# bitmagier/q-learning

Hardware: AMD Instinct MI355X
Metric: env-steps/sec + grad-updates/sec, Breakout 84×84×4, 1/2/4/8 MI355X (higher is better)
Workload: dtype fp32; 1 GPU; C3: 8192 Breakout envs per GPU, replay 1000000 per GPU in HBM (prefilled), Nature-DQN (3 conv + 2 dense) in fp32, B=1024, update every 128 env-steps per GPU (replay ratio 8 samples/env-step), epsilon-greedy acting; envs_per_gpu=8192, batch=1024, replay_capacity=1000000, update_after_actions=128, parallelism=single, rccl_world=1, global_batch_per_update=1024, env_dtype=fp32 physics, u8 frames, qnet_dtype=fp32 (exact-fp32 MFMA v_mfma_f32_16x16x4_f32)

## Files before the change

q-learning_amd/csrc/qnet32.hip:

```cpp
#include <hip/hip_ext.h>
#include <hip/hip_runtime.h>

#include <algorithm>
#include <cmath>
#include <cstdlib>
#include <map>
#include <tuple>
#include <vector>

#include "objects.h"
#include "profiler.h"
#include "qnet.h"
#include "qnet32_kernels.h"
#include "update32_dev.h"

namespace qlx {

using namespace q32;

struct F32Net {
  bool bg_rows = true;
  int c1_skip = 1;
  bool update_scheduled = false;
  bool dense_partials = false;
// ... 591 lines not shown
    if (e && atoi(e) > 0) {
      n = atoi(e);
    } else {
      int dev = 0;
      QLX_HIP(hipGetDevice(&dev));
      QLX_HIP(hipDeviceGetAttribute(&n, hipDeviceAttributeMultiprocessorCount, dev));
    }
  }
  return n;
}

static Grid grid(int M, int BM, int N, int BN, int nz) { return Grid{(M + BM - 1) / BM, (N + BN - 1) / BN, nz}; }

static int c1_skip(const qlx_model* m) { return m->fp32->c1_skip; }

static int balanced_whole_tiles(int M) {
  const int ncu = num_cus(), t = M / 64, whole = t - t % ncu;
  if (whole < ncu || M - whole * 64 > 32 * ncu) return 0;
  return whole;
}

template <class P, class S>
static void launch_list(qlx_model* m, const P& p, const S& side, const char* scope, double work, hipStream_t s) {
  hipEvent_t ea = nullptr, eb = nullptr;
  if (m->prof) m->prof->ext(scope, work, &ea, &eb);
  const size_t lds = std::max(gemm_lds_bytes<P>(), S::LDS);
  hipExtLaunchKernelGGL((k_gemm32_side<P, S>), dim3(side.blocks() + p.g.blocks()), dim3(threads_of<P>()), lds, s, ea, eb, 0u, p, side);
  QLX_HIP(hipGetLastError());
  debug_sync(s, scope);
}

static bool bg_rows(const qlx_model* m) { return m->fp32->bg_rows; }

static bool c1_sparse_dz(const qlx_model* m) { return bg_rows(m) && c1_skip(m); }
template <class PW, class PR, class PF>
static void conv_fwd(qlx_model* m, int M, const float* in, const float* wt, const float* bias, float* out, const char* scope,
                     double work, hipStream_t s, const PF& plain) {
  const int whole = balanced_whole_tiles(M);
  if (!whole) {
    launch(m, plain, scope, work, s);
    return;
  }
  const PW pw{Grid{whole, 1, 1}, in, wt, bias, out, M};
  const PR pr{{Grid{(M - whole * 64 + 15) / 16, 1, 1}, in, wt, bias, out, M}, whole * 4};
  launch_pair(m, pw, pr, NoSide{}, scope, work, s);
}

void f32_forward(qlx_model* m, const uint8_t* const* table, int B, hipStream_t s) {
  F32Net& w = *m->fp32;
  QLX_CHECK(m->ws_batch >= B, QLX_E_STATE, "f32 forward: workspace too small");
  m->last_batch = B;
  const float* p = m->d_params;
  for (int c0 = 0; c0 < B; c0 += w.fchunk) {
    const int n = std::min(w.fchunk, B - c0);
    const bool big = n > 2048;
    const bool lists = bg_rows(m);
    unsigned long long* cnt = w.frcnt + 2 * kListSlots * kCntStride * w.fparity;
    const bool one = c1_one(n);
    const int G = c1_grid(n);
    const int per_slot = ((G + kListSlots - 1) / kListSlots) * ((n + G - 1) / G);
    const int cap2 = per_slot * 81, cap3 = per_slot * 49;
    QLX_CHECK((size_t)kListSlots * cap2 <= w.frl_cap * 81, QLX_E_STATE, "row lists too small");
    const C1Lists L{lists ? w.frl2 : nullptr, w.frl3, cap2, cap3, cnt, w.frcnt + 2 * kListSlots * kCntStride * (w.fparity ^ 1),
                    w.fbgc, w.fsteps, w.fneed, w.fneed_ld, w.frows2, w.fbg2, w.frows3, w.fbg3};
    if (lists) w.fparity ^= 1;
    {
      const char* sc = big ? "f32_conv1_fwd_big" : "f32_conv1_fwd";
      hipEvent_t ea = nullptr, eb = nullptr;
      if (m->prof) m->prof->ext(sc, 2.0 * n * 400 * 32 * 256, &ea, &eb);
      auto kern = one ? k_conv1_fwd32<0, true> : k_conv1_fwd32<1>;
      QLX_CHECK((n + G - 1) / G <= (one ? 1 : kC1MaxIt), QLX_E_STATE, "conv1 forward: too many samples per block");
      const size_t frames = (one ? 1 : 2) * kC1Frames;
      const size_t lds = frames + 3 * kC1RmDw * 4 + (size_t)((n + G - 1) / G) * 6 * 8 + 8;
      set_lds_limit((const void*)kern, frames + 3 * kC1RmDw * 4 + (size_t)(one ? 1 : kC1MaxIt) * 6 * 8 + 8);
      hipExtLaunchKernelGGL(kern, dim3(G), dim3(256), lds, s, ea, eb, 0u, table + (size_t)c0 * 4, n,
                            p + var_offset(0), p + var_offset(1), w.fa1, c1_skip(m), L);
      QLX_HIP(hipGetLastError());
      debug_sync(s, sc);
    }
    if (lists) {
      const int nw = std::min(256, std::max(16, n / 16));
      float* c2 = w.fbgc + 32;
      float* c3 = w.fbgc + 96;
      const BgRows2 s23{{nw, w.frl2, cnt, cap2, c2, w.fa2}, {nw, w.frl3, cnt + kCntStride, cap3, c3, w.fa3}};
      auto lgrid = [&](int cap, int BM, int BN) { return Grid{1 + kListSlots * ((cap + BM - 1) / BM), 64 / BN, 1}; };
      auto run = [&](auto t2, auto t3, const char* sc2, const char* sc3) {
        using P2 = decltype(t2);
        using P3 = decltype(t3);
        const ConstRows cr{{w.fbgc, p + var_offset(2), p + var_offset(3), c2}, {c2, p + var_offset(4), p + var_offset(5), c3}};
        P2 p2{lgrid(cap2, P2::BM, P2::BN), w.fa1, p + var_offset(2), p + var_offset(3), w.fa2, w.frl2, cap2, cnt, w.fbgc};
        p2.pre_batched = big;
        launch_list(m, p2, cr, sc2, 2.0 * n * 81 * 64 * 512, s);
        launch_list(m, P3{lgrid(cap3, P3::BM, P3::BN), w.fa2, p + var_offset(4), p + var_offset(5), w.fa3, w.frl3, cap3, cnt + kCntStride, c2},
                    s23, sc3, 2.0 * n * 49 * 64 * 576, s);
      };
      if (big) {
        run(PConv2FwdL<64, 64, 2, 2>{}, PConv3FwdL<64, 64, 2, 2>{}, "f32_conv2_fwd_big", "f32_conv3_fwd_big");
        launch(m, PFc1FwdB{grid(n, PFc1FwdB::BM, 512, PFc1FwdB::BN, 1), w.fa3, p + var_offset(6), p + var_offset(7), w.fa4 + (size_t)c0 * 512, n}, "f32_fc1_fwd_big",
               2.0 * n * 3136 * 512, s);
      } else {
        run(PConv2FwdL<64, 64, 2, 2>{}, PConv3FwdL<32, 64, 2, 2>{}, "f32_conv2_fwd", "f32_conv3_fwd");
        launch(m, PFc1FwdS{grid(n, PFc1FwdS::BM, 512, PFc1FwdS::BN, 1), w.fa3, p + var_offset(6), p + var_offset(7), w.fa4 + (size_t)c0 * 512, n}, "f32_fc1_fwd",
               2.0 * n * 3136 * 512, s);
      }
    } else if (big) {
      launch(m, PConv2Fwd{grid(n * 81, 64, 64, 64, 1), w.fa1, p + var_offset(2), p + var_offset(3), w.fa2, n * 81}, "f32_conv2_fwd_big",
             2.0 * n * 81 * 64 * 512, s);
      launch(m, PConv3Fwd{grid(n * 49, 64, 64, 64, 1), w.fa2, p + var_offset(4), p + var_offset(5), w.fa3, n * 49}, "f32_conv3_fwd_big",
             2.0 * n * 49 * 64 * 576, s);
      launch(m, PFc1FwdB{grid(n, PFc1FwdB::BM, 512, PFc1FwdB::BN, 1), w.fa3, p + var_offset(6), p + var_offset(7), w.fa4 + (size_t)c0 * 512, n}, "f32_fc1_fwd_big",
             2.0 * n * 3136 * 512, s);
    } else {
      conv_fwd<PConv2Fwd, PConv2FwdR>(m, n * 81, w.fa1, p + var_offset(2), p + var_offset(3), w.fa2, "f32_conv2_fwd", 2.0 * n * 81 * 64 * 512, s,
                                      PConv2FwdS{grid(n * 81, 64, 64, 32, 1), w.fa1, p + var_offset(2), p + var_offset(3), w.fa2, n * 81});
      conv_fwd<PConv3Fwd, PConv3FwdR>(m, n * 49, w.fa2, p + var_offset(4), p + var_offset(5), w.fa3, "f32_conv3_fwd", 2.0 * n * 49 * 64 * 576, s,
                                      PConv3FwdS{grid(n * 49, 64, 64, 32, 1), w.fa2, p + var_offset(4), p + var_offset(5), w.fa3, n * 49});
      launch(m, PFc1FwdS{grid(n, PFc1FwdS::BM, 512, PFc1FwdS::BN, 1), w.fa3, p + var_offset(6), p + var_offset(7), w.fa4 + (size_t)c0 * 512, n}, "f32_fc1_fwd",
             2.0 * n * 3136 * 512, s);
    }
  }
}

void f32_head(int mode, const Fc2Args& a, int B, hipStream_t s) {
  constexpr int kHs3 = 4;
  const dim3 g((B + 15) / 16), blk(256);
  switch (mode) {
    case 0: hipLaunchKernelGGL(k_head32<0>, g, blk, 0, s, a); break;
    case 1: hipLaunchKernelGGL(k_head32<1>, g, blk, 0, s, a); break;
    case 2: hipLaunchKernelGGL(k_head32<2>, g, blk, 0, s, a); break;
    default: hipLaunchKernelGGL((k_head32<3, kHs3>), dim3((B + kHs3 - 1) / kHs3), blk, 0, s, a); break;
  }
  QLX_HIP(hipGetLastError());
  debug_sync(s, "k_head32");
}

Fc2Args f32_fc2_args(qlx_model* m, int B) {
  Fc2Args a = fc2_common(m, B);
  a.a4f = m->fp32->fa4;
  return a;
}

template <class Side>
static void f32_fc1_bwd(qlx_model* m, int B, const Side& S, hipStream_t s) {
  F32Net& w = *m->fp32;
  float* G = m->d_grads;
  const float* p = m->d_params;
  PFc1WgradS Pw{grid(3136, PFc1WgradS::BM, 512, PFc1WgradS::BN, 1), w.fa3, w.fdz4, G + var_offset(6), G + var_offset(7), B};
  PFc1DgradS Pd{grid(B, PFc1DgradS::BM, 3136, PFc1DgradS::BN, 1), w.fdz4, p + var_offset(6), w.fa3, w.fdz3, B};
  if (bg_rows(m)) {
    Pd.pbg = w.fpbg3;
    Pd.bg = w.fbg3;
    Pd.bg_ld = w.fneed_ld;
  }
  launch_pair(m, Pw, Pd, S, "f32_fc1_bwd", 2.0 * 2.0 * B * 512 * 3136, s);
}

void f32_backward_dense(qlx_model* m, int B, const uint8_t* actions, const float* y, float* loss_dev, hipStream_t s,
                        const float* weights, float* td_abs) {
  F32Net& w = *m->fp32;
  QLX_CHECK(B <= w.fchunk && B == m->last_batch, QLX_E_STATE, "f32 backward: batch must follow its forward");
  w.dense_partials = false;
  f32_grad_workspace(m, B);
  float* G = m->d_grads;
  float *gs = m->w.gs, *hs = m->w.hs;
  {
    ProfScope ps(m->prof, "f32_head", s);
    Fc2Args a = f32_fc2_args(m, B);
    a.actions = actions;
    a.y = y;
    a.gsample = gs;
    a.hsample = hs;
    a.weights = weights;
    a.td_abs = td_abs;
    a.dz4_out = w.fdz4;
    f32_head(3, a, B, s);
  }
  f32_fc1_bwd(m, B, SideFc2{w.fa4, actions, gs, hs, B, G + var_offset(8), G + var_offset(9), loss_dev}, s);
}

const float* f32_a4(qlx_model* m) { return m->fp32->fa4; }

float* f32_dz4_begin(qlx_model* m, int B) {
  F32Net& w = *m->fp32;
  QLX_CHECK(B <= w.fchunk && B == m->last_batch, QLX_E_STATE, "f32 backward: batch must follow its forward");
// ... 251 lines not shown
```

q-learning_amd/csrc/qnet32_kernels.h:

```cpp
#pragma once
#include <hip/hip_runtime.h>

#include <cstdint>
#include <type_traits>

#include "qlx_internal.h"

namespace qlx {
namespace q32 {

typedef float f32x4 __attribute__((ext_vector_type(4)));

constexpr int BK = 32;
constexpr int kListSlots = 8;
constexpr int kCntStride = 16;

__host__ __device__ constexpr int kmaj_pad(int rows, int r) { return rows + ((r - rows % 64) % 64 + 64) % 64; }
__host__ __device__ constexpr int kmaj_pitch(int rows) {
  return kmaj_pad(rows, 48) < kmaj_pad(rows, 16) ? kmaj_pad(rows, 48) : kmaj_pad(rows, 16);
}
static_assert(kmaj_pitch(32) == 48 && kmaj_pitch(64) == 80 && kmaj_pitch(128) == 144, "KMAJ pitches");

template <int ROWS, bool KMAJ>
struct Opnd {
// ... 462 lines not shown
      }
    }
  }
}

template <class P>
__device__ __forceinline__ void body(const P& p, int lb, float* lds) { gemm_body(p, lb, lds); }

template <class P>
__global__ __launch_bounds__(threads_of<P>()) void k_gemm32(const P p) {
  extern __shared__ float lds[];
  body(p, block_order<P>(blockIdx.x, gridDim.x), lds);
}

constexpr int kPairMinW = 4;
template <class P, class = void>
struct MinWOf : std::integral_constant<int, 1> {};
template <class P>
struct MinWOf<P, std::void_t<decltype(P::MINW)>> : std::integral_constant<int, P::MINW> {};
template <class P, class = void>
struct HasMinW : std::false_type {};
template <class P>
struct HasMinW<P, std::void_t<decltype(P::MINW)>> : std::true_type {};
template <class P1, class P2>
constexpr int pair_minw() {
  return (HasMinW<P1>::value || HasMinW<P2>::value)
             ? (MinWOf<P1>::value > MinWOf<P2>::value ? MinWOf<P1>::value : MinWOf<P2>::value)
             : kPairMinW;
}
template <class P1, class P2, class S, class T>
__global__ __launch_bounds__(256, (pair_minw<P1, P2>())) void k_gemm32_pair(const P1 p1, const P2 p2, const S side, const T tail) {
  static_assert(KSplitOf<P1>::value == 1 && KSplitOf<P2>::value == 1, "pair launches: 256 threads");
  extern __shared__ float lds[];
  const int b = blockIdx.x, ns = side.blocks();
  if (b < ns) { side.run(b, lds); return; }
  const int h = b - ns;
  const int g1 = p1.g.blocks(), g2 = p2.g.blocks();
  if (h < g1) body(p1, block_order<P1>(h, g1), lds);
  else if (h < g1 + g2) body(p2, block_order<P2>(h - g1, g2), lds);
  else tail.run(h - g1 - g2, lds);
}

template <class P, class S>
__global__ __launch_bounds__(threads_of<P>()) void k_gemm32_side(const P p, const S side) {
  extern __shared__ float lds[];
  const int b = blockIdx.x, ns = side.blocks();
  if (b < ns) { side.run(b, lds); return; }
  body(p, block_order<P>(b - ns, (int)gridDim.x - ns), lds);
}

template <int P = 81>
struct SideBgSum {
  static constexpr size_t LDS = 4 * 64 * sizeof(float);
  static constexpr int Q = (P + 3) / 4;
  const float* pbg;
  float* S;
  int nz;
  __host__ __device__ int blocks() const { return nz; }
  __device__ void run(int z, float* lds) const {
    const int oc = threadIdx.x & 63, q = threadIdx.x >> 6, p0 = Q * q, n = q < 3 ? Q : P - 3 * Q;
    float v[Q];
#pragma unroll
    for (int i = 0; i < Q; ++i) v[i] = i < n ? pbg[((size_t)z * P + p0 + i) * 64 + oc] : 0.0f;
    float t = 0.0f;
#pragma unroll
    for (int i = 0; i < Q; ++i)
      if (i < n) t = __fadd_rn(t, v[i]);
    lds[q * 64 + oc] = t;
    __syncthreads();
    if (q == 0) S[(size_t)z * 64 + oc] = __fadd_rn(__fadd_rn(__fadd_rn(lds[oc], lds[64 + oc]), lds[128 + oc]), lds[192 + oc]);
  }
};

struct NoSide {
  static constexpr size_t LDS = 0;
  __host__ __device__ int blocks() const { return 0; }
  __device__ void run(int, float*) const {}
};


#define QLX_CONV_FWD_CHAINS 1
constexpr int kConvFwdChains = QLX_CONV_FWD_CHAINS;
static_assert(kConvFwdChains == 1, "conv forward policies: one chain per output");
template <int W, int C, int KS, int OC, int BM, int BN, int T, bool SEL = false>
struct ConvFwdStreams {
  using SA = AffineStream<BM, false, T>;
  using SB = AffineStream<BN, true, T>;
  SA a;
  SB b;
  uint32_t cxo[SA::N], msk[SA::N];
  struct Regs {
    typename SA::Regs a;
    typename SB::Regs b;
  };
  __device__ void load(int s, Regs& x) const {
    const int tap = (s * BK) / C, c0 = (s * BK) % C, kh = tap / KS, kw = tap - kh * KS;
    const uint32_t so = (uint32_t)((kh * W + kw) * C + c0) * 4u;
    if constexpr (SEL) {
#pragma unroll
      for (int i = 0; i < SA::N; ++i)
        if (SA::O::F4 % T == 0 || a.tid + i * T < SA::O::F4) {
          const bool cst = (msk[i] >> tap) & 1u;
          x.a[i] = buf_ld4(a.rs, cst ? cxo[i] + (uint32_t)c0 * 4u : a.vo[i] + so, 0u);
        }
    } else {
      a.load(so, 0, x.a);
    }
    b.load((uint32_t)s * BK * OC * 4u, 0, x.b);
  }
  __device__ void store(float* as, float* bs, const Regs& x) const {
    a.store(as, x.a);
    b.store(bs, x.b);
  }
  __device__ void init_b(const float* w, int col0, int tid) {
    b.init(w, (uint32_t)KS * KS * C * OC * 4u, tid, [col0](int r, int k) { return (uint32_t)(k * OC + col0 + r) * 4u; });
  }
};

template <int H, int W, int C, int KS, int S, int OH, int OW, int OC, int BM_ = 64, int BN_ = 64, int WM_ = 2, int WN_ = 2>
struct PConvFwd {
  static constexpr int BM = BM_, BN = BN_, WM = WM_, WN = WN_;
  static constexpr int MINW = 3;
  static constexpr bool LOAD_FENCE = !(H == 20 && BN_ == 64);
  static constexpr bool A_KMAJ = false, B_KMAJ = true, BIAS = false;
  Grid g;
  const float* in;
  const float* w;
  const float* bias;
  float* out;
  int M;
  __host__ __device__ void decode(int lb, int& tm, int& tn, int& z) const { g.decode(lb, tm, tn, z); }
  __host__ __device__ int nslabs(int) const { return KS * KS * C / BK; }
  using Streams = ConvFwdStreams<W, C, KS, OC, BM_, BN_, WM_ * WN_ * 64>;
  __device__ Streams streams(int, int row0, int col0, int tid) const {
    Streams st;
    const int m = M;
    st.a.init(in, (uint32_t)(M / (OH * OW)) * (uint32_t)(H * W * C * 4), tid, [row0, m](int r, int k) {
      const int row = row0 + r, b = row / (OH * OW), p = row - b * (OH * OW), oh = p / OW, ow = p - oh * OW;
      return row < m ? (uint32_t)(((b * H + oh * S) * W + ow * S) * C + k) * 4u : kOob;
    });
    st.init_b(w, col0, tid);
    return st;
  }
  __device__ void epi(int, int row, int col, f32x4 v) const {
#pragma unroll
    for (int r = 0; r < 4; ++r)
      if (row + r < M) out[(size_t)(row + r) * OC + col] = relu(v[r] + bias[col]);
  }
  __device__ f32x4 epi_pre(int, int, int col) const {
    const float b = bias[col];
    return f32x4{b, b, b, b};
  }
  __device__ void epi_post(int, int row, int col, f32x4 v, f32x4 b) const {
#pragma unroll
    for (int r = 0; r < 4; ++r)
      if (row + r < M) out[(size_t)(row + r) * OC + col] = relu(v[r] + b[r]);
  }
};
using PConv2Fwd = PConvFwd<20, 20, 32, 4, 2, 9, 9, 64>;
using PConv3Fwd = PConvFwd<9, 9, 64, 3, 1, 7, 7, 64>;
using PConv2FwdS = PConvFwd<20, 20, 32, 4, 2, 9, 9, 64, 64, 32, 2, 2>;
using PConv3FwdS = PConvFwd<9, 9, 64, 3, 1, 7, 7, 64, 64, 32, 2, 2>;
template <class Base>
struct RowShift : Base {
  int tm0;
  __host__ __device__ void decode(int lb, int& tm, int& tn, int& z) const {
    Base::decode(lb, tm, tn, z);
    tm += tm0;
  }
};
using PConv2FwdR = RowShift<PConvFwd<20, 20, 32, 4, 2, 9, 9, 64, 16, 64, 1, 4>>;
using PConv3FwdR = RowShift<PConvFwd<9, 9, 64, 3, 1, 7, 7, 64, 16, 64, 1, 4>>;

template <int H, int W, int C, int KS, int S, int OH, int OW, int OC, int BM_ = 64, int BN_ = 64, int WM_ = 2, int WN_ = 2,
          bool SEL = false>
struct PConvFwdL {
  static constexpr int BM = BM_, BN = BN_, WM = WM_, WN = WN_;
  static constexpr bool A_KMAJ = false, B_KMAJ = true, BIAS = false, RAW_ORDER = true;
  static constexpr bool LOAD_FENCE = true;
  static constexpr int R = OH * OW;
  using OA = Opnd<BM, false>;
  static constexpr int T = WM * WN * 64, NA = (OA::F4 + T - 1) / T;
  Grid g;
  const float* in;
  const float* w;
  const float* bias;
  float* out;
  const int* list;
  int cap;
  const unsigned long long* cnt;
  const float* cx;
  bool pre_batched = true;
  struct Pre { float b; int o[4]; };

  __host__ __device__ void decode(int lb, int& tm, int& tn, int& z) const { g.decode(lb, tm, tn, z); }
  __host__ __device__ int nslabs(int) const { return KS * KS * C / BK; }
  __device__ int count(int x) const { return (int)(cnt[x * 2 * kCntStride] >> 32); }
  template <int N>
  __device__ void entries(const int (&row)[N], int (&out)[N]) const {
    const int tm = q32_uniform(row[0] / BM);
    const int x = (tm - 1) % kListSlots, base = ((tm - 1) / kListSlots) * BM;
    const int n = count(x);
    int v[N];
#pragma unroll
    for (int i = 0; i < N; ++i) v[i] = list[x * cap + min(base + row[i] % BM, cap - 1)];
#pragma unroll
    for (int i = 0; i < N; ++i) out[i] = base + row[i] % BM < n ? v[i] : -1;
  }
  __device__ bool active(int, int row0) const {
    const int tm = row0 / BM;
    return tm != 0 && ((tm - 1) / kListSlots) * BM < count((tm - 1) % kListSlots);
  }
  __device__ Pre epi_pre(int, int row, int col) const {
    Pre q;
    q.b = bias[col];
    if (!pre_batched) {
#pragma unroll
    for (int r = 0; r < 4; ++r) {
      const int tm = (row + r) / BM;
      const int x = (tm - 1) % kListSlots, lr = ((tm - 1) / kListSlots) * BM + (row + r) % BM;
      q.o[r] = lr < count(x) ? list[x * cap + lr] : -1;
    }
    } else {
    const int rows[4] = {row, row + 1, row + 2, row + 3};
    entries(rows, q.o);
    }
    return q;
  }
  __device__ void epi_post(int, int, int col, f32x4 v, const Pre& q) const {
#pragma unroll
    for (int r = 0; r < 4; ++r)
      if (q.o[r] >= 0) out[(size_t)(q.o[r] & 0xFFFFF) * OC + col] = relu(v[r] + q.b);
  }
  using Streams = ConvFwdStreams<W, C, KS, OC, BM_, BN_, T, SEL>;
  __device__ Streams streams(int, int row0, int col0, int tid) const {
    Streams st;
    st.a.tid = tid;
    const char* lo = (const char*)in;
    const char* base = SEL && (const char*)cx < lo ? (const char*)cx : lo;
    const uint32_t in_off = (uint32_t)(lo - base), cx_off = SEL ? (uint32_t)((const char*)cx - base) : 0u;
    st.a.rs = buf_rsrc(base, kNoEnd);
    int rows[NA], raws[NA];
#pragma unroll
    for (int i = 0; i < NA; ++i) {
      int r = 0, k = 0;
      OA::coord(tid + i * T, r, k);
      rows[i] = row0 + r;
    }
    entries(rows, raws);
#pragma unroll
    for (int i = 0; i < NA; ++i) {
      int r = 0, k = 0;
      OA::coord(tid + i * T, r, k);
      const int raw = raws[i], e = raw >= 0 ? raw & 0xFFFFF : -1;
      const int bb = e / R, pp = e - bb * R, oh = pp / OW, ow = pp - oh * OW;
      st.a.vo[i] = e >= 0 ? in_off + (uint32_t)(((bb * H + oh * S) * W + ow * S) * C + k) * 4u : kOob;
      st.cxo[i] = cx_off + (uint32_t)k * 4u;
      st.msk[i] = SEL && raw >= 0 ? (uint32_t)raw >> 20 : 0u;
    }
    st.init_b(w, col0, tid);
    return st;
  }
};
template <int BM, int BN, int WM, int WN>
using PConv2FwdL = PConvFwdL<20, 20, 32, 4, 2, 9, 9, 64, BM, BN, WM, WN, false>;
template <int BM, int BN, int WM, int WN>
using PConv3FwdL = PConvFwdL<9, 9, 64, 3, 1, 7, 7, 64, BM, BN, WM, WN, true>;

template <int C, int KS, int OC>
struct PConstRow {
  static constexpr int BM = 16, BN = OC, WM = 1, WN = 4, T = 256;
  static constexpr bool A_KMAJ = false, B_KMAJ = true, BIAS = false;
  static constexpr Grid g{1, 1, 1};
  const float* cx;
  const float* w;
  const float* bias;
  float* cbuf;
  __host__ __device__ void decode(int, int& tm, int& tn, int& z) const { tm = tn = z = 0; }
  __host__ __device__ int nslabs(int) const { return KS * KS * C / BK; }
  __device__ float epi_pre(int, int, int col) const { return bias[col]; }
  __device__ void epi_post(int, int row, int col, f32x4 v, float b) const {
    if (row == 0) cbuf[col] = relu(v[0] + b);
  }
  struct Streams {
    AffineStream<BM, false, T> a;
    AffineStream<BN, true, T> b;
    struct Regs {
      typename AffineStream<BM, false, T>::Regs a;
      typename AffineStream<BN, true, T>::Regs b;
    };
    __device__ void load(int s, Regs& x) const {
      a.load((uint32_t)((s * BK) % C) * 4u, 0, x.a);
      b.load((uint32_t)s * BK * OC * 4u, 0, x.b);
    }
    __device__ void store(float* as, float* bs, const Regs& x) const {
      a.store(as, x.a);
      b.store(bs, x.b);
    }
  };
  __device__ Streams streams(int, int, int, int tid) const {
    Streams st;
    st.a.init(cx, (uint32_t)C * 4u, tid, [](int r, int k) { return r == 0 ? (uint32_t)k * 4u : kOob; });
    st.b.init(w, (uint32_t)KS * KS * C * OC * 4u, tid, [](int r, int k) { return (uint32_t)(k * OC + r) * 4u; });
    return st;
  }
};

struct ConstRows {
  using PA = PConstRow<32, 4, 64>;
  using PB = PConstRow<64, 3, 64>;
  static constexpr size_t LDS = gemm_lds_bytes<PA>();
  PA pa;
  PB pb;
  __host__ __device__ int blocks() const { return 1; }
  __device__ void run(int, float* lds) const {
    gemm_body(pa, 0, lds);
    __syncthreads();
    __threadfence();
    gemm_body(pb, 0, lds);
  }
};

struct BgRows {
  static constexpr size_t LDS = 64 * sizeof(float);
  static constexpr int U = 8;
  int nblk;
  const int* list;
  const unsigned long long* cnt;
  int cap;
  const float* c_in;
  float* out;
  __host__ __device__ int blocks() const { return nblk; }
  __device__ void run(int blk, float* lds) const {
    const int tid = threadIdx.x, q = tid & 15, RB = (int)blockDim.x >> 4;
    const f32x4 v = ld4(c_in + 4 * q);
    for (int x = 0; x < kListSlots; ++x) {
      const int nbg = (int)(uint32_t)cnt[x * 2 * kCntStride];
      const int* back = list + (size_t)(x + 1) * cap - 1;
      for (int i0 = blk * RB * U + (tid >> 4); i0 < nbg; i0 += nblk * RB * U) {
        int e[U];
#pragma unroll
        for (int u = 0; u < U; ++u) e[u] = i0 + RB * u < nbg ? back[-(i0 + RB * u)] : -1;
#pragma unroll
        for (int u = 0; u < U; ++u)
          if (e[u] >= 0) *reinterpret_cast<f32x4*>(out + (size_t)e[u] * 64 + 4 * q) = v;
      }
    }
  }
};
struct BgRows2 {
  static constexpr size_t LDS = BgRows::LDS;
  BgRows a, b;
  __host__ __device__ int blocks() const { return a.nblk + b.nblk; }
  __device__ void run(int blk, float* lds) const {
    if (blk < a.nblk) a.run(blk, lds);
    else b.run(blk - a.nblk, lds);
  }
};

#define QLX_FC1_CHAINS 2
constexpr int kFc1Chains = QLX_FC1_CHAINS;
template <int BM_, int BN_, int WM_, int WN_, int KS_ = 1, int KQ_ = kFc1Chains>
struct PFc1FwdT {
  static constexpr int BM = BM_, BN = BN_, WM = WM_, WN = WN_;
  static constexpr int KSPLIT = KS_, KSEQ = KQ_;
  static_assert(KS_ * KQ_ == kFc1Chains, "fc1 forward: the chain definition");
  static constexpr bool LOAD_FENCE = false;
  static constexpr int IGLP = BM_ == 64 ? 1 : 0;
  static constexpr bool A_KMAJ = false, B_KMAJ = true, BIAS = false;
  Grid g;
  const float* a3;
  const float* w3;
  const float* b3;
  float* a4;
  int M;
  __host__ __device__ void decode(int lb, int& tm, int& tn, int& z) const { g.decode(lb, tm, tn, z); }
  __host__ __device__ int nslabs(int) const { return 3136 / BK; }
  __device__ void epi(int, int row, int col, f32x4 v) const {
#pragma unroll
    for (int r = 0; r < 4; ++r)
      if (row + r < M) a4[(size_t)(row + r) * 512 + col] = relu(v[r] + b3[col]);
  }
  __device__ f32x4 epi_pre(int, int, int col) const {
    const float b = b3[col];
    return f32x4{b, b, b, b};
  }
  __device__ void epi_post(int, int row, int col, f32x4 v, f32x4 b) const {
#pragma unroll
    for (int r = 0; r < 4; ++r)
      if (row + r < M) a4[(size_t)(row + r) * 512 + col] = relu(v[r] + b[r]);
  }
  static constexpr int T = WM_ * WN_ * 64;
  using SA = AffineStream<BM_, false, T>;
  using SB = AffineStream<BN_, true, T>;
  using Streams = PairStreams<SA, SB, BK * 4u, BK * 512u * 4u>;
  __device__ Streams streams(int, int row0, int col0, int tid) const {
    Streams st;
    const int m = M;
    st.a.init(a3, (uint32_t)M * 3136u * 4u, tid,
              [row0, m](int r, int k) { return row0 + r < m ? (uint32_t)((row0 + r) * 3136 + k) * 4u : kOob; });
    st.b.init(w3, 3136u * 512u * 4u, tid, [col0](int r, int k) { return (uint32_t)(k * 512 + col0 + r) * 4u; });
    st.kmax = 3136;
    return st;
  }
};
using PFc1FwdB = PFc1FwdT<64, 128, 2, 2, 1, kFc1Chains>;
using PFc1FwdS = PFc1FwdT<32, 32, 2, 2, kFc1Chains, 1>;

#ifndef QLX_Q32_POLICIES_ONLY
__device__ __forceinline__ float pb_sum16(const float (&d)[4]) {
  float s = __fadd_rn(__fadd_rn(__fadd_rn(d[0], d[1]), d[2]), d[3]);
  const auto r16 = __builtin_amdgcn_permlane16_swap(__float_as_uint(s), __float_as_uint(s), false, false);
  s = __fadd_rn(__uint_as_float(r16[0]), __uint_as_float(r16[1]));
  const auto r32 = __builtin_amdgcn_permlane32_swap(__float_as_uint(s), __float_as_uint(s), false, false);
  return __fadd_rn(__uint_as_float(r32[0]), __uint_as_float(r32[1]));
}
#else
inline float pb_sum16(const float (&d)[4]) { return ((d[0] + d[1]) + d[2]) + d[3]; }
#endif

template <int BM_, int BN_, int WM_, int WN_>
struct PFc1DgradT {
  static constexpr int BM = BM_, BN = BN_, WM = WM_, WN = WN_;
  static constexpr bool A_KMAJ = false, B_KMAJ = false, BIAS = false;
  Grid g;
  const float* dz4;
  const float* w3;
  const float* a3;
  float* dz3;
  int M;
  float* pbg = nullptr;
  const uint8_t* bg = nullptr;
  int bg_ld = 0;
  struct Pre {
    f32x4 m;
    uint32_t bg;
  };
  __host__ __device__ void decode(int lb, int& tm, int& tn, int& z) const { g.decode(lb, tm, tn, z); }
  __host__ __device__ int nslabs(int) const { return 512 / BK; }
// ... 590 lines not shown
    nd[h] = valid && ((((rm[oh] | rm[oh + 1]) >> (4 * t)) & 0x1Fu) != 0u);
    if (need && valid) need[(size_t)s * need_ld + b] = nd[h] ? 1 : 0;
  }
  const unsigned long long m0 = __builtin_amdgcn_ballot_w64(nd[0]), m1 = __builtin_amdgcn_ballot_w64(nd[1]);
  if (lane < 4) {
    const unsigned long long m = lane < 2 ? m0 : m1;
    out[lane] = (uint32_t)(m >> (32 * (lane & 1)));
  }
}
__device__ __forceinline__ bool c1_step_set(unsigned long long lo, unsigned long long hi, int st) {
  return ((st < 64 ? lo >> st : hi >> (st - 64)) & 1ull) != 0ull;
}
__device__ __forceinline__ uint32_t c1_tiles(const uint32_t* rm, int lane) {
  const int t = lane < 25 ? lane : 0, bx = 4 * (t / 5), by = 4 * (t % 5);
  uint32_t mm = 0;
#pragma unroll
  for (int r = 0; r < 5; ++r) mm |= rm[bx + r];
  return (uint32_t)__builtin_amdgcn_ballot_w64(lane < 25 && ((mm >> by) & 0x1Fu) != 0u);
}
__device__ __forceinline__ void c1_flags(const uint32_t* rm, unsigned long long* cl, int wave, const C1Lists& L, int b) {
  const int tid = c1_opaque_tid();
  const int R = wave < 2 ? 81 : 49, p = wave < 2 ? tid : tid - 128;
  const bool valid = p < R;
  const int pp = valid ? p : 0;
  bool nonbg;
  if (wave < 2) {
    const int i = pp / 9, j = pp - 9 * i;
    uint32_t mm = 0;
#pragma unroll
    for (int r = 0; r < 5; ++r) mm |= rm[2 * i + r];
    nonbg = ((mm >> (2 * j)) & 0x1Fu) != 0u;
  } else {
    const int i = pp / 7, j = pp - 7 * i;
    uint32_t mm = 0;
#pragma unroll
    for (int r = 0; r < 9; ++r) mm |= rm[2 * i + r];
    nonbg = ((mm >> (2 * j)) & 0x1FFu) != 0u;
  }
  const unsigned long long bn = __builtin_amdgcn_ballot_w64(valid && nonbg), bb = __builtin_amdgcn_ballot_w64(valid && !nonbg);
  if ((tid & 63) == 0) {
    cl[0] = bn;
    cl[1] = bb;
  }
  if (wave < 2 && L.rows2) {
    const int lane = tid & 63;
    if (lane < 2 && (wave == 0 || lane == 0)) L.rows2[(size_t)b * 4 + 2 * wave + lane] = (uint32_t)(bn >> (32 * lane));
    if (wave == 1 && lane == 1) L.rows2[(size_t)b * 4 + 3] = 0u;
    if (valid) L.bg2[(size_t)p * L.need_ld + b] = nonbg ? 0 : 1;
  }
  if (wave == 2 && L.rows3) {
    const int lane = tid & 63;
    if (lane < 4) L.rows3[(size_t)b * 4 + lane] = lane < 2 ? (uint32_t)(bn >> (32 * lane)) : 0u;
    if (valid) L.bg3[(size_t)p * L.need_ld + b] = nonbg ? 0 : 1;
  }
}
__device__ __forceinline__ void c1_lists_flush(const unsigned long long* cl, int nit, int b0, int G, const C1Lists& L, int wave,
                                               int tid, unsigned long long* xch) {
  const int lane = tid & 63, R = wave < 2 ? 81 : 49, p = wave < 2 ? tid : tid - 128;
  int* rl = wave < 2 ? L.rl2 : L.rl3;
  auto wave_tot = [&](int wv) {
    unsigned long long t = 0;
    for (int it = 0; it < nit; ++it)
      t += ((unsigned long long)__builtin_popcountll(cl[(it * 3 + wv) * 2]) << 32) |
           (unsigned long long)__builtin_popcountll(cl[(it * 3 + wv) * 2 + 1]);
    return t;
  };
  unsigned long long old = 0;
  const int slot = blockIdx.x % kListSlots, cap = wave < 2 ? L.cap2 : L.cap3;
  rl += slot * cap;
  if ((wave == 0 || wave == 2) && lane == 0) {
    const unsigned long long tot = wave == 0 ? wave_tot(0) + wave_tot(1) : wave_tot(2);
    old = __hip_atomic_fetch_add(L.cnt + (slot * 2 + (wave < 2 ? 0 : 1)) * kCntStride, tot, __ATOMIC_RELAXED, __HIP_MEMORY_SCOPE_AGENT);
    if (wave == 0) *xch = old;
  }
  __syncthreads();
  if (wave == 1) old = *xch + wave_tot(0);
  if (wave >= 3) return;
  old = __shfl(old, 0);
  int on = (int)(old >> 32), og = (int)(uint32_t)old;
  const unsigned long long below = (1ull << lane) - 1ull;
  for (int it = 0; it < nit; ++it) {
    const unsigned long long bn = cl[(it * 3 + wave) * 2], bb = cl[(it * 3 + wave) * 2 + 1];
    const int e = (b0 + it * G) * R + p;
    int tap = 0;
    if (wave == 2) {
      const unsigned long long g0 = cl[(it * 3) * 2 + 1], g1 = cl[(it * 3 + 1) * 2 + 1];
      const int i = p / 7, j = p - 7 * (p / 7);
#pragma unroll
      for (int t = 0; t < 9; ++t) {
        const int q = (i + t / 3) * 9 + j + t % 3;
        tap |= (int)(((q < 64 ? g0 >> q : g1 >> (q - 64)) & 1ull) << t);
      }
    }
    if ((bn >> lane) & 1ull) rl[on + __builtin_popcountll(bn & below)] = e | (tap << 20);
    else if ((bb >> lane) & 1ull) rl[cap - 1 - (og + __builtin_popcountll(bb & below))] = e;
    on += __builtin_popcountll(bn);
    og += __builtin_popcountll(bb);
  }
}

__device__ __forceinline__ void c1_fwd_sample(const uint32_t* fr, uint32_t lb, int nt, int rp, int g, int col,
                                              const float (&wf)[64], float bias, int skip, uint32_t live, float* a1, int b) {
  {
    const unsigned long long every = skip == 0 ? ~0ull : 0ull;
    auto tile_live = [&](int j) { return ((live >> (rp + 2 * j)) & 1u) != 0u; };
    auto tile_dwords = [&](int j, uint32_t (&d)[16]) {
      const int t = rp + 2 * j;
      const uint32_t base = lb + (uint32_t)((t / 5) * (16 * 21) + (t % 5) * 4);
#pragma unroll
      for (int kq = 0; kq < 16; ++kq) d[kq] = fr[base + (kq >> 1) * 21 + (kq & 1)];
    };
    const uint32_t so = (uint32_t)(g * 20 * 32 + col);
    const float zb = relu(0.0f + bias);
    auto tile = [&](int j, const uint32_t (&d)[16], uint32_t (&dn)[16]) {
      const bool lv = tile_live(j), nx = j + 1 < nt && tile_live(j + 1);
      const int t = rp + 2 * j;
      float* at = a1 + ((size_t)b * 400 + 80 * (t / 5) + 4 * (t % 5)) * 32;
      if (lv) {
        bool nz[16];
#pragma unroll
        for (int kq = 0; kq < 16; ++kq) nz[kq] = (__builtin_amdgcn_ballot_w64(d[kq] != 0u) | every) != 0ull;
        if (nx) tile_dwords(j + 1, dn);
        f32x4 acc = zero4();
#pragma unroll
        for (int kq = 0; kq < 16; ++kq)
          if (nz[kq])
#pragma unroll
            for (int kw = 0; kw < 4; ++kw) acc = __builtin_amdgcn_mfma_f32_16x16x4f32(ubyte(d[kq], kw), wf[kq * 4 + kw], acc, 0, 0, 0);
#pragma unroll
        for (int i = 0; i < 4; ++i) at[so + 32u * i] = relu(acc[i] + bias);
      } else {
        if (nx) tile_dwords(j + 1, dn);
#pragma unroll
        for (int i = 0; i < 4; ++i) at[so + 32u * i] = zb;
      }
    };
    uint32_t dd[14][16];
    if (tile_live(0)) tile_dwords(0, dd[0]);
#pragma unroll
    for (int j = 0; j < 13; ++j)
      if (j < nt) tile(j, dd[j], dd[j + 1]);
  }
}

constexpr int kC1OneMinW = 4;
template <int ROLE, bool ONE = false>
__global__ __launch_bounds__(256, ONE ? kC1OneMinW : 2) void k_conv1_fwd32(const uint8_t* const* table, int B, const float* w0,
                                                                           const float* b0, float* a1, int skip, const C1Lists L) {
  extern __shared__ __attribute__((aligned(16))) uint32_t c1w[];
  uint32_t* rm = c1w + (ONE ? 1 : 2) * 4 * kC1SlotDw;
  unsigned long long* cl = reinterpret_cast<unsigned long long*>(rm + 3 * kC1RmDw);
  const bool lists = L.rl2 != nullptr;
  const bool marks = lists || L.rows2 != nullptr || L.rows3 != nullptr;
  const int tid = threadIdx.x, lane = tid & 63;
  const int wave = __builtin_amdgcn_readfirstlane(tid >> 6);
  if (marks) {
    if (blockIdx.x == 0 && tid < 2 * kListSlots) L.cnt_next[tid * kCntStride] = 0ull;
    if (blockIdx.x == 0 && tid < 32) L.xbg[tid] = relu(0.0f + b0[tid]);
    if (tid < 3 * kC1RmDw) rm[tid] = 0u;
    __syncthreads();
  }
  const int ct = wave & 1, rp = wave >> 1;
  const int col = ct * 16 + (lane & 15), g = lane >> 4;
  float wf[64];
#pragma unroll
  for (int kk = 0; kk < 64; ++kk) wf[kk] = w0[(kk * 4 + g) * 32 + col];
  const float bias = b0[col];
  const uint32_t lb = (uint32_t)(g * kC1SlotDw + 4 * ((lane & 15) >> 2) * 21 + (lane & 3));
  const int nt = rp == 0 ? 13 : 12;
  int b = blockIdx.x;
  if (b >= B) return;
  if constexpr (ONE) {
    {
      uint4 pf[7];
      c1_prefetch(c1_ptrs(table, b), pf);
      c1_stage(c1w, pf);
      if (marks) c1_mark(rm, pf);
// ... 186 lines not shown
```

Baseline: 333,500 env-steps/s.

## Drop conv3 tap-select path and move const-row work into conv2 side blocks

Removes the per-tap selection path in the conv3 list kernel. That path used a tap mask packed into the row list, so each A load could pick between the live input and a constant background row. Conv3 rows now always read the conv2 activation buffer, so conv2 must have written the background rows into fa2. The ConstRows side kernel and the BgRows2 pair are replaced by a Conv2Side object: block 0 computes both constant rows, and each other block recomputes the conv2 constant row in LDS and scatters it to the background rows. Conv3 then only scatters its own background rows. This trims the list-building tap computation and the per-load selects in conv3, at the cost of redundant constant-row GEMMs in every scatter block and extra fa2 writes for background positions.

```diff
diff --git a/q-learning_amd/csrc/qnet32.hip b/q-learning_amd/csrc/qnet32.hip
--- a/q-learning_amd/csrc/qnet32.hip
+++ b/q-learning_amd/csrc/qnet32.hip
@@ -697,24 +697,25 @@
       const int nw = std::min(256, std::max(16, n / 16));
       float* c2 = w.fbgc + 32;
       float* c3 = w.fbgc + 96;
-      const BgRows2 s23{{nw, w.frl2, cnt, cap2, c2, w.fa2}, {nw, w.frl3, cnt + kCntStride, cap3, c3, w.fa3}};
+      const Conv2Side s2{{w.fbgc, p + var_offset(2), p + var_offset(3), c2}, {c2, p + var_offset(4), p + var_offset(5), c3},
+                         {nw, w.frl2, cnt, cap2, c2, w.fa2}};
+      const BgRows s3{nw, w.frl3, cnt + kCntStride, cap3, c3, w.fa3};
       auto lgrid = [&](int cap, int BM, int BN) { return Grid{1 + kListSlots * ((cap + BM - 1) / BM), 64 / BN, 1}; };
       auto run = [&](auto t2, auto t3, const char* sc2, const char* sc3) {
         using P2 = decltype(t2);
         using P3 = decltype(t3);
-        const ConstRows cr{{w.fbgc, p + var_offset(2), p + var_offset(3), c2}, {c2, p + var_offset(4), p + var_offset(5), c3}};
-        P2 p2{lgrid(cap2, P2::BM, P2::BN), w.fa1, p + var_offset(2), p + var_offset(3), w.fa2, w.frl2, cap2, cnt, w.fbgc};
+        P2 p2{lgrid(cap2, P2::BM, P2::BN), w.fa1, p + var_offset(2), p + var_offset(3), w.fa2, w.frl2, cap2, cnt};
         p2.pre_batched = big;
-        launch_list(m, p2, cr, sc2, 2.0 * n * 81 * 64 * 512, s);
-        launch_list(m, P3{lgrid(cap3, P3::BM, P3::BN), w.fa2, p + var_offset(4), p + var_offset(5), w.fa3, w.frl3, cap3, cnt + kCntStride, c2},
-                    s23, sc3, 2.0 * n * 49 * 64 * 576, s);
+        launch_list(m, p2, s2, sc2, 2.0 * n * 81 * 64 * 512, s);
+        launch_list(m, P3{lgrid(cap3, P3::BM, P3::BN), w.fa2, p + var_offset(4), p + var_offset(5), w.fa3, w.frl3, cap3, cnt + kCntStride},
+                    s3, sc3, 2.0 * n * 49 * 64 * 576, s);
       };
       if (big) {
-        run(PConv2FwdL<64, 64, 2, 2>{}, PConv3FwdL<64, 64, 2, 2>{}, "f32_conv2_fwd_big", "f32_conv3_fwd_big");
+        run(PConv2FwdL<64, 64, 2, 2, 1>{}, PConv3FwdL<64, 64, 2, 2, 1>{}, "f32_conv2_fwd_big", "f32_conv3_fwd_big");
         launch(m, PFc1FwdB{grid(n, PFc1FwdB::BM, 512, PFc1FwdB::BN, 1), w.fa3, p + var_offset(6), p + var_offset(7), w.fa4 + (size_t)c0 * 512, n}, "f32_fc1_fwd_big",
                2.0 * n * 3136 * 512, s);
       } else {
-        run(PConv2FwdL<64, 64, 2, 2>{}, PConv3FwdL<32, 64, 2, 2>{}, "f32_conv2_fwd", "f32_conv3_fwd");
+        run(PConv2FwdL<64, 64, 2, 2, 0>{}, PConv3FwdL<32, 64, 2, 2, 0>{}, "f32_conv2_fwd", "f32_conv3_fwd");
         launch(m, PFc1FwdS{grid(n, PFc1FwdS::BM, 512, PFc1FwdS::BN, 1), w.fa3, p + var_offset(6), p + var_offset(7), w.fa4 + (size_t)c0 * 512, n}, "f32_fc1_fwd",
                2.0 * n * 3136 * 512, s);
       }
diff --git a/q-learning_amd/csrc/qnet32_kernels.h b/q-learning_amd/csrc/qnet32_kernels.h
--- a/q-learning_amd/csrc/qnet32_kernels.h
+++ b/q-learning_amd/csrc/qnet32_kernels.h
@@ -568,30 +568,19 @@
 #define QLX_CONV_FWD_CHAINS 1
 constexpr int kConvFwdChains = QLX_CONV_FWD_CHAINS;
 static_assert(kConvFwdChains == 1, "conv forward policies: one chain per output");
-template <int W, int C, int KS, int OC, int BM, int BN, int T, bool SEL = false>
+template <int W, int C, int KS, int OC, int BM, int BN, int T>
 struct ConvFwdStreams {
   using SA = AffineStream<BM, false, T>;
   using SB = AffineStream<BN, true, T>;
   SA a;
   SB b;
-  uint32_t cxo[SA::N], msk[SA::N];
   struct Regs {
     typename SA::Regs a;
     typename SB::Regs b;
   };
   __device__ void load(int s, Regs& x) const {
     const int tap = (s * BK) / C, c0 = (s * BK) % C, kh = tap / KS, kw = tap - kh * KS;
-    const uint32_t so = (uint32_t)((kh * W + kw) * C + c0) * 4u;
-    if constexpr (SEL) {
-#pragma unroll
-      for (int i = 0; i < SA::N; ++i)
-        if (SA::O::F4 % T == 0 || a.tid + i * T < SA::O::F4) {
-          const bool cst = (msk[i] >> tap) & 1u;
-          x.a[i] = buf_ld4(a.rs, cst ? cxo[i] + (uint32_t)c0 * 4u : a.vo[i] + so, 0u);
-        }
-    } else {
-      a.load(so, 0, x.a);
-    }
+    a.load((uint32_t)((kh * W + kw) * C + c0) * 4u, 0, x.a);
     b.load((uint32_t)s * BK * OC * 4u, 0, x.b);
   }
   __device__ void store(float* as, float* bs, const Regs& x) const {
@@ -659,7 +648,7 @@
 using PConv3FwdR = RowShift<PConvFwd<9, 9, 64, 3, 1, 7, 7, 64, 16, 64, 1, 4>>;
 
 template <int H, int W, int C, int KS, int S, int OH, int OW, int OC, int BM_ = 64, int BN_ = 64, int WM_ = 2, int WN_ = 2,
-          bool SEL = false>
+          int ROLE = 0>
 struct PConvFwdL {
   static constexpr int BM = BM_, BN = BN_, WM = WM_, WN = WN_;
   static constexpr bool A_KMAJ = false, B_KMAJ = true, BIAS = false, RAW_ORDER = true;
@@ -675,7 +664,6 @@
   const int* list;
   int cap;
   const unsigned long long* cnt;
-  const float* cx;
   bool pre_batched = true;
   struct Pre { float b; int o[4]; };
 
@@ -716,16 +704,13 @@
   __device__ void epi_post(int, int, int col, f32x4 v, const Pre& q) const {
 #pragma unroll
     for (int r = 0; r < 4; ++r)
-      if (q.o[r] >= 0) out[(size_t)(q.o[r] & 0xFFFFF) * OC + col] = relu(v[r] + q.b);
-  }
-  using Streams = ConvFwdStreams<W, C, KS, OC, BM_, BN_, T, SEL>;
+      if (q.o[r] >= 0) out[(size_t)q.o[r] * OC + col] = relu(v[r] + q.b);
+  }
+  using Streams = ConvFwdStreams<W, C, KS, OC, BM_, BN_, T>;
   __device__ Streams streams(int, int row0, int col0, int tid) const {
     Streams st;
     st.a.tid = tid;
-    const char* lo = (const char*)in;
-    const char* base = SEL && (const char*)cx < lo ? (const char*)cx : lo;
-    const uint32_t in_off = (uint32_t)(lo - base), cx_off = SEL ? (uint32_t)((const char*)cx - base) : 0u;
-    st.a.rs = buf_rsrc(base, kNoEnd);
+    st.a.rs = buf_rsrc(in, kNoEnd);
     int rows[NA], raws[NA];
 #pragma unroll
     for (int i = 0; i < NA; ++i) {
@@ -738,20 +723,18 @@
     for (int i = 0; i < NA; ++i) {
       int r = 0, k = 0;
       OA::coord(tid + i * T, r, k);
-      const int raw = raws[i], e = raw >= 0 ? raw & 0xFFFFF : -1;
+      const int e = raws[i];
       const int bb = e / R, pp = e - bb * R, oh = pp / OW, ow = pp - oh * OW;
-      st.a.vo[i] = e >= 0 ? in_off + (uint32_t)(((bb * H + oh * S) * W + ow * S) * C + k) * 4u : kOob;
-      st.cxo[i] = cx_off + (uint32_t)k * 4u;
-      st.msk[i] = SEL && raw >= 0 ? (uint32_t)raw >> 20 : 0u;
+      st.a.vo[i] = e >= 0 ? (uint32_t)(((bb * H + oh * S) * W + ow * S) * C + k) * 4u : kOob;
     }
     st.init_b(w, col0, tid);
     return st;
   }
 };
-template <int BM, int BN, int WM, int WN>
-using PConv2FwdL = PConvFwdL<20, 20, 32, 4, 2, 9, 9, 64, BM, BN, WM, WN, false>;
-template <int BM, int BN, int WM, int WN>
-using PConv3FwdL = PConvFwdL<9, 9, 64, 3, 1, 7, 7, 64, BM, BN, WM, WN, true>;
+template <int BM, int BN, int WM, int WN, int ROLE>
+using PConv2FwdL = PConvFwdL<20, 20, 32, 4, 2, 9, 9, 64, BM, BN, WM, WN, ROLE>;
+template <int BM, int BN, int WM, int WN, int ROLE>
+using PConv3FwdL = PConvFwdL<9, 9, 64, 3, 1, 7, 7, 64, BM, BN, WM, WN, ROLE>;
 
 template <int C, int KS, int OC>
 struct PConstRow {
@@ -792,20 +775,9 @@
   }
 };
 
-struct ConstRows {
-  using PA = PConstRow<32, 4, 64>;
-  using PB = PConstRow<64, 3, 64>;
-  static constexpr size_t LDS = gemm_lds_bytes<PA>();
-  PA pa;
-  PB pb;
-  __host__ __device__ int blocks() const { return 1; }
-  __device__ void run(int, float* lds) const {
-    gemm_body(pa, 0, lds);
-    __syncthreads();
-    __threadfence();
-    gemm_body(pb, 0, lds);
-  }
-};
+using PConstRow2 = PConstRow<32, 4, 64>;
+using PConstRow3 = PConstRow<64, 3, 64>;
+static_assert(gemm_lds_bytes<PConstRow2>() == gemm_lds_bytes<PConstRow3>(), "the constant rows: both 16 x 64 tiles");
 
 struct BgRows {
   static constexpr size_t LDS = 64 * sizeof(float);
@@ -834,13 +806,28 @@
     }
   }
 };
-struct BgRows2 {
-  static constexpr size_t LDS = BgRows::LDS;
-  BgRows a, b;
-  __host__ __device__ int blocks() const { return a.nblk + b.nblk; }
+struct Conv2Side {
+  static constexpr size_t LDS = gemm_lds_bytes<PConstRow2>() + 64 * sizeof(float);
+  PConstRow2 pa;
+  PConstRow3 pb;
+  BgRows bg;
+  __host__ __device__ int blocks() const { return 1 + bg.nblk; }
   __device__ void run(int blk, float* lds) const {
-    if (blk < a.nblk) a.run(blk, lds);
-    else b.run(blk - a.nblk, lds);
+    if (blk == 0) {
+      gemm_body(pa, 0, lds);
+      __syncthreads();
+      __threadfence();
+      gemm_body(pb, 0, lds);
+      return;
+    }
+    float* c2 = lds + gemm_lds_bytes<PConstRow2>() / sizeof(float);
+    PConstRow2 mine = pa;
+    mine.cbuf = c2;
+    gemm_body(mine, 0, lds);
+    __syncthreads();
+    BgRows rows = bg;
+    rows.c_in = c2;
+    rows.run(blk - 1, lds);
   }
 };
 
@@ -1597,17 +1584,7 @@
   for (int it = 0; it < nit; ++it) {
     const unsigned long long bn = cl[(it * 3 + wave) * 2], bb = cl[(it * 3 + wave) * 2 + 1];
     const int e = (b0 + it * G) * R + p;
-    int tap = 0;
-    if (wave == 2) {
-      const unsigned long long g0 = cl[(it * 3) * 2 + 1], g1 = cl[(it * 3 + 1) * 2 + 1];
-      const int i = p / 7, j = p - 7 * (p / 7);
-#pragma unroll
-      for (int t = 0; t < 9; ++t) {
-        const int q = (i + t / 3) * 9 + j + t % 3;
-        tap |= (int)(((q < 64 ? g0 >> q : g1 >> (q - 64)) & 1ull) << t);
-      }
-    }
-    if ((bn >> lane) & 1ull) rl[on + __builtin_popcountll(bn & below)] = e | (tap << 20);
+    if ((bn >> lane) & 1ull) rl[on + __builtin_popcountll(bn & below)] = e;
     else if ((bb >> lane) & 1ull) rl[cap - 1 - (og + __builtin_popcountll(bb & below))] = e;
     on += __builtin_popcountll(bn);
     og += __builtin_popcountll(bb);
```

Result: no change. 334,600 env-steps/s, median of 6 (+0.3%).
